# Forrest-Z/my-lidar-graph-slam

Hardware: AMD Instinct MI355X
Metric: scans/sec + p50 scan-match ms, 1081-beam vs 1000×1000@5cm grid, 1/2/4/8 GPU (higher is better)
Workload: dtype f64

## Files before the change

### include/lgs_hip.h

```cpp
#ifndef LGS_HIP_H
#define LGS_HIP_H

#include <stddef.h>
#include <stdint.h>

#ifdef __cplusplus
extern "C" {
#endif

#define LGS_ABI_VERSION 2

#define LGS_OK               0
#define LGS_ERR_INVALID_ARG  1
#define LGS_ERR_HIP          2
#define LGS_ERR_NO_DEVICE    3
#define LGS_ERR_OOM          4
#define LGS_ERR_INTERNAL     5

typedef struct lgs_ctx  lgs_ctx;
typedef struct lgs_grid lgs_grid;
typedef struct lgs_scan lgs_scan;

typedef struct { double x, y, theta; } lgs_pose2d;

// ... 64 lines not shown
#define LGS_OPT_SORT_BARRIER_US 23
#define LGS_OPT_FINE_STAGED   24
#define LGS_OPT_SMALL_WINDOW  25
#define LGS_OPT_POST_RECORDS  26
#define LGS_OPT_FUSED_PLANES  27
#define LGS_OPT_PRIORITY_TAIL 28
#define LGS_OPT_HV_FULL       29
#define LGS_OPT_SPLIT_CHUNKS  30
#define LGS_OPT_DEVICE_HITS   31
#define LGS_OPT_SEED_WIDE     32
#define LGS_OPT_ZERO_TILES    33
#define LGS_OPT_DEVICE_TIMING 34
#define LGS_OPT_LEAN_PROJECT  35
#define LGS_OPT_PGCG_GRID_NODES 36
#define LGS_OPT_FAST_ROWS     37
#define LGS_OPT_HV_INZERO     38
#define LGS_OPT_POISON_WS     15
int  lgs_ctx_set_option(lgs_ctx* ctx, int option, double value);

int  lgs_debug_item_buffer(lgs_ctx* ctx, int item, int which, void* out, size_t cap, size_t* bytes);

int  lgs_debug_libm(lgs_ctx* ctx, int op, const double* x, int n, double* out);

int  lgs_debug_keysort(lgs_ctx* ctx, const unsigned* keys, unsigned* out, long long n, int lo, int bits);

int  lgs_debug_copy_counters(const lgs_ctx* ctx, long long* direct, long long* staged);

int  lgs_debug_offset_checks(lgs_ctx* ctx, int reset, unsigned long long* out);

typedef struct {
// ... 468 lines not shown
```

### my-lidar-graph-slam_amd/csrc/k_rtcsm.hip

```cpp
#include "lgs_internal.hpp"
#include "loop_host.hpp"
#include "fast_cell.hpp"
#include "hv_zero.hpp"
#include "sq_cost_stage.hpp"
#include "ge_cost_device.hpp"

#include <algorithm>
#include <cfloat>
#include <cstring>
#include <map>
#include <mutex>
#include <thread>
#include <type_traits>

using namespace lgs;

namespace lgs {
void launch_precompute(lgs_ctx* ctx, const lgs_grid* in, int win, double* out, const PlaneGeom* planes);
void launch_precompute_jobs(lgs_ctx* ctx, const PrecompJob* d_jobs, int njobs, int maxW, int maxH, int win);
bool precompute_planes_ok(const lgs_grid* in, int win);
void precompute_tile_grid(int maxW, int maxH, int win, int njobs, int* gx, int* gy, int* rows);
}

namespace {
// ... 14 lines not shown
    const double* cmap;
    const SuperT* super;
    const int* negflag;
    int pgen;
    int gen;
    RtcsmRecord* rec;
    int* keepc;
    int2* idx;
    int* cbase;
    int* tedge;
    double* cscore;
    uint8_t* cflag;
    int* list;
    int* segcnt;
    int nseg;
    int* dlist;
    int* nsel;
    int frows;
    double* fval;
    int* fpos;
    double* part_c;
    long long* part_k;
    int nparts;
    double* Lp;
    double* Lc;
    double* seedm;
    int nseedm;
    double* sbound;
    double* poses7;
    int4* cidx;
// ... 1561 lines not shown
                    if (q.x - pl.win_x < 0 || q.y - pl.win_y < 0)
                        unsafe |= strip_read(cmap, q.x + x0, q.y + y0, pl, ext);
                }
            }
        }
        if (active) {
            it.cflag[k] = (unsafe && (sum + ext) * pl.sb_mult >= L) ? 1 : 0;
        }
    }
}

struct WorkList {
    int* cnt;
    int* sbl;
    int* al;
    int region, tmax;
};
constexpr int kListMaxNv = 4096;
#ifndef LGS_LIST_WAVES
#define LGS_LIST_WAVES 4096
#endif
constexpr int kListWaves = LGS_LIST_WAVES;
#ifndef LGS_LIST_XCD
#define LGS_LIST_XCD 1
#endif
#ifndef LGS_XCD2
#define LGS_XCD2 1
#endif
static_assert(kListWaves % 8 == 0, "whole workgroups per XCD");
constexpr int kUnsafeGroups = 4096;

__global__ __launch_bounds__(64) void k_keep(Items items, WorkList W, DevTs dts)
// ... 4 lines not shown
    const RtcsmPlan& pl = it.pl;
    const int t = blockIdx.x;
    if (t >= pl.T) return;
    const int lane = threadIdx.x;
    const int nsb2 = pl.nsbx * pl.nsby;
    double L = -INFINITY;
#pragma unroll
    for (int b = 0; b < kSeedCands; ++b) L = fmax(L, it.Lc[b]);
    if (t == 0 && lane == 0) *it.Lp = L;
    bool kp = false;
    if (lane < nsb2) {
        const double bnd = it.sbound[(size_t)t * nsb2 + lane];
        kp = (bnd > pl.thr) && bnd >= L;
    }
    const unsigned long long bal = __ballot(kp);
    if (!bal) return;
    int base = 0;
    if (lane == 0) {
        unsigned long long nb = 0;
        for (unsigned long long mm = bal; mm; mm &= mm - 1) {
            const int sb = __ffsll((long long)mm) - 1;
            const int a = sb % pl.nsbx, b = sb / pl.nsbx;
            nb += (unsigned long long)(min(kSB, pl.ncx - kSB * a) * min(kSB, pl.ncy - kSB * b));
        }
        atomicAdd(&it.rec->coarse_evals, nb);
        base = atomicAdd(W.cnt + 16 * j, __popcll(bal));
        if (it.tedge[t] == it.gen) W.al[(size_t)j * W.tmax + atomicAdd(W.cnt + 16 * j + 1, 1)] = t;
    }
    base = __shfl(base, 0, 64);
    if (kp) W.sbl[(size_t)j * W.region + base + __popcll(bal & ((1ull << lane) - 1ull))] = t << 6 | lane;
}

__device__ __forceinline__ int list_prefix(const WorkList& W, int which, int n, int& c)
{
    const int lane = threadIdx.x & 63;
    c = lane < n ? W.cnt[16 * lane + which] : 0;
#pragma unroll
    for (int off = 1; off < 64; off <<= 1) {
        const int u = __shfl_up(c, off, 64);
        if (lane >= off) c += u;
    }
    return __shfl(c, 63, 64);
// ... 109 lines not shown
        }
        if (active) {
            const long long k = (long long)t * pl.P + (long long)jx * pl.ncy + jy;
            it.cscore[k] = sum;
            it.cflag[k] = 0;
        }
    }
}

__global__ __launch_bounds__(64 * kLaneWaves) void k_unsafe_list(Items items, WorkList W, int n,
                                                                 const double* __restrict__ zero, DevTs dts)
{
    const DtsScope dts_scope(dts);
    const int lane = threadIdx.x & 63;
    int c;
    const int total = list_prefix(W, 1, n, c);
    for (int a = blockIdx.x; a < total; a += gridDim.x) {
        const int j = __popcll(__ballot(lane < n && c <= a));
        const int cprev = __shfl(c, max(j - 1, 0), 64);
        const int before = j > 0 ? cprev : 0;
        unsafe_angle(items[j], W.al[(size_t)j * W.tmax + (a - before)]);
    }
}

__device__ void eval_block(const RtcsmPlan& pl, const double* __restrict__ grid,
                           const int2* __restrict__ idx, const double* __restrict__ zero,
                           long long k, int2* sidx, double& f, int& pos)
{
    const int tt = (int)(k / pl.P);
    const int rem = (int)(k % pl.P);
    const int jx = rem / pl.ncy, jy = rem % pl.ncy;
// ... 324 lines not shown
            if (k[r] == bk) v[r] = -INFINITY, k[r] = LLONG_MAX;
    }
    return pick;
}
__global__ __launch_bounds__(kSeedMembersThreads) void k_seed_members(Items items, DevTs dts)
{
#if LGS_XCD2
    const Blk sbk = xcd_block();
#else
    const Blk sbk{ (int)blockIdx.x, (int)blockIdx.y, (int)blockIdx.z };
#endif
    const DtsScope dts_scope(dts);
    const MatchItem& it = items[sbk.y];
    const RtcsmPlan& pl = it.pl;
    const double* __restrict__ cmap = it.cmap;
    if (sbk.x == 0 && threadIdx.x < 2 && it.keepc) it.keepc[threadIdx.x] = 0;
    extern __shared__ char smem[];
    __shared__ double red[2][kSeedMembersThreads / 64][16];
    __shared__ long long s_cand;
    const int tid = threadIdx.x, lane = tid & 63, w = tid >> 6;
    const int nsb2 = pl.nsbx * pl.nsby;
    const int Nv = pl.Nv;
    if (w == 0) {
        const long long pick = seed_pick_wave(it, pl, (int)sbk.x);
        if (lane == 0) s_cand = pick;
    }
    __syncthreads();
    double* out = it.seedm + 3 * sbk.x;
    const long long ck = s_cand;
    if (ck == LLONG_MAX) {
        if (tid == 0) {
// ... 79 lines not shown
#if LGS_XCD2
    const Blk sbk = xcd_block();
#else
    const Blk sbk{ (int)blockIdx.x, (int)blockIdx.y, (int)blockIdx.z };
#endif
    const DtsScope dts_scope(dts);
    const MatchItem& it = items[sbk.y];
    const RtcsmPlan& pl = it.pl;
    const double* __restrict__ grid = it.grid;
    const double* __restrict__ cmap = it.cmap;
    const double* __restrict__ part_c = it.part_c;
    const long long* __restrict__ part_k = it.part_k;
    const int nparts = it.nparts;
    double* __restrict__ Lc = it.Lc;
    RtcsmRecord* rec = it.rec;
    if (MODE == 0 && sbk.x == 0 && threadIdx.x < 2 && it.keepc) it.keepc[threadIdx.x] = 0;
    extern __shared__ char smem[];
    __shared__ double sv[16];
    __shared__ long long sk[16];
    __shared__ long long cand[kSeedCands];
    __shared__ double red[1024];
    __shared__ double reda[1024];
    const int tid = threadIdx.x;
    const int nsb2 = pl.nsbx * pl.nsby;
    const int Nv = pl.Nv;
    LGS_PROBE_DECL;
    LGS_PROBE_MARK();
    double Lmine = -INFINITY;
    if constexpr (MODE == 2) {
        if (tid < 64) {
            const bool ok = tid < it.nseedm;
// ... 152 lines not shown
            }
        }
        __syncthreads();
        Lmine = seed_fine(pl, grid, zero, sidx, sk[0], sv[1], sv[2], red, reda, sv);
        LGS_PROBE_MARK();
    }
    if (tid == 0) {
        Lc[sbk.x] = Lmine;
        if (sbk.x == 0) rec->coarse_evals = 0ull;
    }
    LGS_PROBE_MARK();
    LGS_PROBE_PRINT("seed(b0: cand, members, argmax, stage, fine, reduce, publish)");
}

constexpr int kSelSeg = 1024;

template <int kSelThreads>
__global__ __launch_bounds__(kSelThreads) void k_select(Items items, int use_sbound, DevTs dts)
{
    const DtsScope dts_scope(dts);
    static_assert(kSelSeg % kSelThreads == 0 && kSelThreads % 64 == 0, "whole chunks of whole waves");
    const MatchItem& it = items[blockIdx.y];
    if ((int)blockIdx.x >= it.nseg) return;
    const RtcsmPlan& pl = it.pl;
    const double* __restrict__ cscore = it.cscore;
    const uint8_t* __restrict__ cflag = it.cflag;
    const double* __restrict__ sbound = use_sbound ? it.sbound : nullptr;
    int* __restrict__ list = it.list;
    int* __restrict__ segcnt = it.segcnt;
    constexpr int kW = kSelThreads / 64, kChunks = kSelSeg / kSelThreads;
    __shared__ int s_w[kChunks][kW];
    const double L = *it.Lp;
    const int lane = threadIdx.x & 63, wid = threadIdx.x >> 6;
    bool f[kChunks];
#pragma unroll
    for (int j = 0; j < kChunks; ++j) {
// ... 22 lines not shown
        const unsigned long long bal = __ballot(f[j]);
        int o = off;
        for (int w = 0; w < wid; ++w) o += s_w[j][w];
        if (f[j]) list[(size_t)blockIdx.x * kSelSeg + o + __popcll(bal & ((1ull << lane) - 1ull))] =
            (int)((long long)blockIdx.x * kSelSeg + j * kSelThreads + threadIdx.x);
        for (int w = 0; w < kW; ++w) off += s_w[j][w];
    }
    if (threadIdx.x == 0) segcnt[blockIdx.x] = off;
}

__device__ void seg_prefix(const int* __restrict__ segcnt, int nseg, int* pref, int* ws)
{
    const int nt = blockDim.x, tid = threadIdx.x, lane = tid & 63, wid = tid >> 6;
    const int chunk = (nseg + nt - 1) / nt;
    const int lo = min(tid * chunk, nseg), hi = min(lo + chunk, nseg);
    int c = 0;
    for (int i = lo; i < hi; ++i) c += segcnt[i];
    int incl = c;
    for (int off = 1; off < 64; off <<= 1) {
        const int t = __shfl_up(incl, off, 64);
        if (lane >= off) incl += t;
    }
    const int last = min(63, nt - 1 - wid * 64);
    if (lane == last) ws[wid] = incl;
    __syncthreads();
    int run = incl - c;
    for (int j = 0; j < wid; ++j) run += ws[j];
    for (int i = lo; i < hi; ++i) {
        pref[i] = run;
        run += segcnt[i];
    }
    if (tid == nt - 1) pref[nseg] = run;
    __syncthreads();
}

__device__ __forceinline__ int seg_of(const int* pref, int nseg, int b)
{
    int lo = 0, hi = nseg;
    while (hi - lo > 1) {
        const int mid = (lo + hi) >> 1;
        if (pref[mid] <= b) lo = mid;
        else hi = mid;
    }
    return lo;
}
// ... 14 lines not shown
    int* __restrict__ fpos = it_.fpos;
    extern __shared__ char smem[];
    __shared__ double sv[16];
    __shared__ long long sk[16];
    __shared__ int ws[16];
    int* pref = (int*)(smem + eval_smem);
    LGS_PROBE_DECL;
    LGS_PROBE_MARK();
    seg_prefix(segcnt, nseg, pref, ws);
    LGS_PROBE_MARK();
    const int n = pref[nseg];
    constexpr int R = LR > 0 ? LR : 1;
    for (int it = wg.x; it < n * R; it += gridDim.x) {
        const int b = it / R;
        const int sg = seg_of(pref, nseg, b);
        const long long k = list[(size_t)sg * kSelSeg + (b - pref[sg])];
        double f;
        int pos;
        if constexpr (LR > 0)
            eval_block_t<LR, kFineDepth>(pl, grid, idx, zero, k, smem, sv, sk, f, pos, it % R);
        else
            eval_block(pl, grid, idx, zero, k, (int2*)smem, f, pos);
        if (threadIdx.x == 0) {
            fval[it] = f;
            fpos[it] = pos;
        }
        LGS_PROBE_MARK();
    }
    LGS_PROBE_PRINT("fine(seg_prefix, item0[, item1])");
}

__global__ __launch_bounds__(256) void k_compact(Items items)
{
    const MatchItem& it = items[blockIdx.x];
    extern __shared__ int pref[];
    __shared__ int ws[16];
    seg_prefix(it.segcnt, it.nseg, pref, ws);
    const int lane = threadIdx.x & 63, w = threadIdx.x >> 6;
    for (int sg = w; sg < it.nseg; sg += 4) {
        const int c = pref[sg + 1] - pref[sg];
        const int* __restrict__ src = it.list + (size_t)sg * kSelSeg;
        int* __restrict__ dst = it.dlist + pref[sg];
        for (int i = lane; i < c; i += 64) dst[i] = src[i];
    }
    if (threadIdx.x == 0) *it.nsel = pref[it.nseg];
}

constexpr int kFineLanesWaves = 1;
constexpr int kFineLanesMaxNv = 2048;
__global__ __launch_bounds__(64 * kFineLanesWaves) void k_fine_lanes(Items items, int n,
                                                                    const double* __restrict__ zero)
{
    __shared__ int ipref[kMaxBatchItems + 1];
    extern __shared__ int2 sidx[];
    if (threadIdx.x < 64) {
        const int j = threadIdx.x;
        const int c = (j < n) ? *items[j].nsel : 0;
        int incl = c;
        for (int off = 1; off < 64; off <<= 1) {
            const int t = __shfl_up(incl, off, 64);
// ... 208 lines not shown
    seg_prefix(segcnt, nseg, pref, ws);
    const int n = pref[nseg];
    const double L = *Lp;
    const int lane = threadIdx.x;
    double s = pl.thr;
    long long bestk = -1;
    int bestpos = 0;
    bool dangerous = false;
    for (int b0 = 0; b0 < n; b0 += 64) {
        const int b = b0 + lane;
        double c = -INFINITY, f = -INFINITY;
        long long k = -1;
        int pos = 0;
        if (b < n) {
            const int sg = seg_of(pref, nseg, b);
            k = list[(size_t)sg * kSelSeg + (b - pref[sg])];
            c = cscore[k];
            const size_t fi = (size_t)b * frows;
            f = fval[fi];
            pos = fpos[fi];
            for (int r = 1; r < frows; ++r) {
                const double fr = fval[fi + r];
                const int pr = fpos[fi + r];
                if (fr > f || (fr == f && pr < pos)) {
                    f = fr;
                    pos = pr;
                }
            }
            if (cflag[k] && c < L && f >= L) dangerous = true;
        }
        const int cnt = min(64, n - b0);
// ... 753 lines not shown
    int P = 0, nsb2 = 0, chunks = 0, low_res = 0, cb = 0;
    bool pair = false;
    bool oct = false;
    int unit8 = 2;
    int nsby = 0;
    bool pruned = false;
    bool small = false;
    bool lr5 = false;
    bool fine_lanes = false;
    bool fine_staged = false;
    int frows = 1;
    int kernel_size = 0;
    bool sq = false;
    bool gx = false;
    WorkList wl{};
};

inline int item_nparts(const BatchShape& B, const RtcsmPlan& pl, bool pruned)
{
    return pruned ? B.chunks * pl.T : ((B.P + B.cb - 1) / B.cb) * pl.T;
}

inline bool uses_super(const lgs_ctx* ctx, int nv_max, int nsb2, bool dense)
{
    return !(dense || ctx->force_dense) && ctx->super_prune && nv_max <= kSeedMaxNv &&
           nsb2 <= 64 && nsb2 >= ctx->prune_min_super;
}

struct ItemLayout {
    size_t idx, cbase, cscore, cflag, list, segcnt, dlist, fval, fpos, part_c, part_k, sbound, poses7, cidx,
        terms, count, btab, atab, total;
};
ItemLayout item_layout(int Tmax, int NvMax, int P, int nsb2, int chunks, int cb, int frows, int Nmax)
{
    ItemLayout L{};
    size_t o = 0;
    auto take = [&](size_t bytes) {
        const size_t r = o;
        o += align256(std::max<size_t>(bytes, 16));
        return r;
    };
    const size_t K = (size_t)Tmax * P;
    const size_t nidx = (size_t)Tmax * std::max(NvMax, 1) + kPad;
    const size_t nseg = (K + kSelSeg - 1) / kSelSeg;
    const size_t nparts = std::max<size_t>((size_t)((P + cb - 1) / cb) * Tmax, (size_t)chunks * Tmax);
    L.idx = take(sizeof(int2) * nidx);
    L.cbase = take(sizeof(int) * 2 * nidx);
    L.cscore = take(sizeof(double) * K);
    L.cflag = take(K);
    L.list = take(sizeof(int) * nseg * kSelSeg);
    L.segcnt = take(sizeof(int) * nseg);
    L.dlist = take(sizeof(int) * K);
    L.fval = take(sizeof(double) * K * frows);
    L.fpos = take(sizeof(int) * K * frows);
    L.part_c = take(sizeof(double) * nparts);
    L.part_k = take(sizeof(long long) * nparts);
    L.sbound = take(sizeof(double) * (size_t)Tmax * std::max(nsb2, 1));
    L.poses7 = take(sizeof(double) * 21);
    L.cidx = take(sizeof(int4) * 7 * (size_t)Nmax);
    L.terms = take(sizeof(double) * 7 * (size_t)Nmax);
    L.count = take(128 + 24 * kSeedWide);
    L.btab = take(sizeof(double4) * (size_t)std::max(NvMax, 1));
    L.atab = take(sizeof(double2) * (size_t)std::max(Tmax, 1));
    L.total = o;
    return L;
}

void bind_workspace(MatchItem& it, char* base, const ItemLayout& L, int frows)
{
    it.idx = (int2*)(base + L.idx);
    it.cbase = (int*)(base + L.cbase);
    it.cscore = (double*)(base + L.cscore);
    it.cflag = (uint8_t*)(base + L.cflag);
    it.list = (int*)(base + L.list);
    it.segcnt = (int*)(base + L.segcnt);
    it.fval = (double*)(base + L.fval);
    it.fpos = (int*)(base + L.fpos);
    it.part_c = (double*)(base + L.part_c);
    it.part_k = (long long*)(base + L.part_k);
    it.sbound = (double*)(base + L.sbound);
    it.poses7 = (double*)(base + L.poses7);
    it.cidx = (int4*)(base + L.cidx);
    it.terms = (double*)(base + L.terms);
    it.Lp = (double*)(base + L.count);
    it.Lc = (double*)(base + L.count + 64);
    it.nsel = (int*)(base + L.count + 64 + 8 * kSeedCands);
    it.seedm = (double*)(base + L.count + 128);
    it.dlist = (int*)(base + L.dlist);
    it.btab = (double4*)(base + L.btab);
    it.atab = (double2*)(base + L.atab);
    static_assert(64 + 8 * kSeedCands + 4 <= 128, "count block layout");
    it.frows = frows;
    it.nseg = (int)((it.pl.K + kSelSeg - 1) / kSelSeg);
}

inline size_t plane_bytes(const RtcsmPlan& pl)
{
    return align256(sizeof(double) * (size_t)pl.low_res * pl.low_res * (size_t)pl.pstride);
}
inline size_t plane16_bytes(const RtcsmPlan& pl)
{
    return align256(sizeof(unsigned short) * (size_t)pl.low_res * pl.low_res * (size_t)pl.pstride) + 256;
}
inline size_t set_bytes(const RtcsmPlan& pl) { return plane_bytes(pl) + plane16_bytes(pl); }
inline size_t super_bytes(const RtcsmPlan& pl)
{
    if (pl.oct) return align256(4 * (size_t)pl.unit8 * pl.low_res * pl.low_res * (size_t)pl.pstrideO);
    return align256(sizeof(SuperT) * (size_t)pl.low_res * pl.low_res * (size_t)pl.pstride4);
// ... 557 lines not shown
            ctx->timing_end(tok);
            LGS_HIP_CHECK(hipGetLastError());
        }
        const int tok = ctx->timing_begin(K_SEED, 8.0 * B.low_res * B.low_res * (double)B.NvMax * n);
        if (B.lr5)
            hipLaunchKernelGGL(k_seed<5>, dim3(1, n), dim3(64 * 5), eval_t_smem<5>(B.NvMax), st, d_items, zero,
                               dense ? 1 : 0);
        else
            hipLaunchKernelGGL(k_seed<0>, dim3(1, n), dim3(64), sidx_bytes(B.NvMax), st, d_items, zero,
                               dense ? 1 : 0);
        ctx->timing_end(tok);
        LGS_HIP_CHECK(hipGetLastError());
    }
    {
        const int tok_ = ctx->timing_begin(K_SELECT, 10.0 * (double)B.Tmax * B.P * n);
        if (!ctx->skipped(K_SELECT)) {
            if (n >= ctx->lanes_min_batch)
                hipLaunchKernelGGL(HIP_KERNEL_NAME(k_select<256>), dim3((unsigned)B.nsegMax, n), dim3(256), 0, st,
                                   d_items, B.pruned ? 1 : 0, ctx->dts(tok_));
            else
                hipLaunchKernelGGL(HIP_KERNEL_NAME(k_select<kSelSeg>), dim3((unsigned)B.nsegMax, n), dim3(kSelSeg), 0,
                                   st, d_items, B.pruned ? 1 : 0, ctx->dts(tok_));
        }
        ctx->timing_end(tok_);
        LGS_HIP_CHECK(hipGetLastError());
    }
    if (B.fine_lanes) {
        hipLaunchKernelGGL(k_compact, dim3(n), dim3(256), pref_bytes(B.nsegMax), st, d_items);
        LGS_HIP_CHECK(hipGetLastError());
        const int tok_ = ctx->timing_begin(K_FINE, 0.0);
        if (ctx->skipped(K_FINE)) {
        } else if (B.fine_staged && ctx->fine_staged) {
            hipLaunchKernelGGL(k_fine_regs, dim3(4096), dim3(64), sizeof(unsigned) * (size_t)(B.NvMax + kFrPad), st,
                               d_items, n, zero, ctx->dts(tok_));
        } else {
            hipLaunchKernelGGL(k_fine_lanes, dim3(4096), dim3(64 * kFineLanesWaves),
                               sizeof(int2) * (size_t)(B.NvMax + 4 * kPipe), st, d_items, n, zero);
// ... 292 lines not shown
    B.oct = p0.oct != 0;
    B.unit8 = p0.unit8;
    B.nsby = p0.nsby;
    B.pruned = uses_super(ctx, B.NvMax, B.nsb2, false);
    B.lr5 = lr5_path(B.NvMax, B.low_res);
    B.fine_lanes = n >= ctx->lanes_min_batch && B.low_res * B.low_res <= 64 &&
                   B.NvMax <= kFineLanesMaxNv;
    B.frows = (B.lr5 && !B.fine_lanes) ? 5 : 1;
    B.fine_staged = B.fine_lanes && B.low_res == 5;
    for (int j = 0; j < n && B.fine_staged; ++j)
        B.fine_staged = grids[j]->w % 2 == 0 && ((uintptr_t)grids[j]->d & 15) == 0 && grids[j]->w <= 8192 &&
                        grids[j]->h <= 8192;
    B.kernel_size = cost->kernel_size;
    B.sq = sq != nullptr;
    B.gx = alt.gx;
    B.nsegMax = (int)(((long long)B.Tmax * B.P + kSelSeg - 1) / kSelSeg);
    B.small = ctx->small_window && !ctx->force_dense && p0.P == 1 && B.low_res >= 2 && B.low_res <= 7 &&
              B.NvMax <= kSmallMaxNv && n <= kTedgeCtrs;
    for (int j = 0; j < n; ++j) B.small = B.small && grids[j]->w >= B.low_res && grids[j]->h >= 1;
    for (auto& s : sets) B.small = B.small && !s.coarse;
    if (B.small) B.pruned = false;
    if (B.pruned && n >= ctx->lanes_min_batch && B.NvMax <= kListMaxNv && B.Tmax < (1 << 24) && B.nsb2 <= 64) {
        int region = 1;
        for (auto& it : items) region = std::max(region, it.pl.T * it.pl.nsbx * it.pl.nsby);
        int* wl = (int*)ctx->ensure(S_KEEP, sizeof(int) * (size_t)n * (16 + (size_t)region + (size_t)B.Tmax));
        B.wl = WorkList{ wl, wl + 16 * (size_t)n, wl + 16 * (size_t)n + (size_t)region * n, region, B.Tmax };
    }
    const ItemLayout L = item_layout(B.Tmax, B.NvMax, B.P, B.nsb2, B.chunks, B.cb, B.frows, Nmax);
    char* ws = (char*)ctx->ensure(ctx->banked(S_BATCH_WS), L.total * (size_t)n);
    RtcsmRecord* d_rec = (RtcsmRecord*)ctx->ensure(ctx->banked(S_RECORDS), sizeof(RtcsmRecord) * (size_t)n);
    const size_t rec_bytes = sizeof(RtcsmRecord) * (size_t)n;
    constexpr size_t kDtsBytes = sizeof(unsigned long long) * 2 * kDtsSub * kDtsSlots;
    RtcsmRecord* h_rec = (RtcsmRecord*)ctx->ensure_pinned_rec(align256(rec_bytes) + 256 + kDtsBytes);
    unsigned* h_flag = (unsigned*)((char*)h_rec + align256(rec_bytes));
    F.id = ++ctx->timing_batch;
    struct DtsScope {
        lgs_ctx* c;
        ~DtsScope() { c->dts_dev = nullptr; }
    } dts_scope{ ctx };
    if (ctx->profile && ctx->dev_timing) {
        unsigned long long*& db = ctx->dts_buf[ctx->bank];
        if (++ctx->dts_gen >= (1u << 24) || !db) {
// ... 8 lines not shown
        ctx->dts_used = 0;
    }
    if (ctx->poison_ws) {
        LGS_HIP_CHECK(hipMemsetAsync(ws, 0xFF, L.total * (size_t)n, ctx->stream));
        LGS_HIP_CHECK(hipMemsetAsync(d_rec, 0xFF, sizeof(RtcsmRecord) * (size_t)n, ctx->stream));
    }
    int* tedge = ctx->tedge_buffer((size_t)n * B.Tmax);
    int* sctr = B.small ? ctx->small_counters((size_t)n * B.Tmax) : nullptr;
    Upload up(ctx);
    scans_to_device(ctx, scans, n, &up);
    const SetJobs sj = B.small ? SetJobs{} : build_sets(ctx, p0, sets, B.pruned, up);
    std::vector<int> gens((size_t)n);
    for (int j = 0; j < n; ++j) {
        MatchItem& it = items[j];
        bind_workspace(it, ws + L.total * (size_t)j, L, B.frows);
        it.tedge = tedge + (size_t)j * B.Tmax;
        it.grid = grids[j]->d;
        it.ranges = scans[j]->d_ranges;
        it.angles = scans[j]->d_angles;
        const PlaneSet& s = sets[set_of[j]];
        it.cmap = s.cmap;
        it.super = s.super;
        it.negflag = s.negflag;
        it.pgen = s.pgen;
        it.gen = gens[j] = ctx->generation = ctx->next_stamp();
        it.rec = d_rec + j;
        it.keepc = B.wl.cnt ? B.wl.cnt + 16 * j : sctr ? sctr + j : nullptr;
        it.nparts = item_nparts(B, it.pl, B.pruned);
        it.nseedm = std::min(ctx->seed_wide, kSeedWide);
        it.inject = ctx->inject_index ? 1 : 0;
// ... 15 lines not shown
                               sizeof(int2) * (size_t)q.T * q.Nv, sizeof(double) * (size_t)q.K };
        lgs_ctx::DbgItem& d = ctx->dbg[j];
        for (int k = 0; k < 8; ++k) {
            d.buf[k] = b[k];
            d.bytes[k] = sz[k];
        }
        d.buf[8] = ij.cmap;
        d.bytes[8] = ij.cmap ? plane_bytes(q) : 0;
        d.buf[9] = ij.super;
        d.bytes[9] = ij.super ? super_bytes(q) : 0;
        const PlaneSet* dps = B.small ? nullptr : &sets[set_of[j]];
        d.buf[10] = dps ? dps->hv_in : nullptr;
        d.bytes[10] = dps ? dps->hv_in_bytes : 0;
        d.buf[11] = dps ? dps->hv_out : nullptr;
        d.bytes[11] = dps ? dps->hv_out_bytes : 0;
        d.gen = ij.gen;
    }
    const size_t items_off = up.append(items.data(), items.size());
    up.flush();
    if (!B.small) launch_sets(ctx, p0, sets, sj, up);
    struct StreamRestore {
        lgs_ctx* c;
        hipStream_t s;
        ~StreamRestore() { c->stream = s; }
    } restore{ ctx, ctx->stream };
    if (!B.small && ctx->prio_tail && ctx->hi) {
        LGS_HIP_CHECK(hipEventRecord(ctx->split_ev[ctx->bank], ctx->stream));
        LGS_HIP_CHECK(hipStreamWaitEvent(ctx->hi, ctx->split_ev[ctx->bank], 0));
        ctx->stream = ctx->hi;
    }
// ... 110 lines not shown
                                host_cost_cells(cp, scans[j], P7[pi], b, cells);
                                cpatch.push_back(make_int4(pi * cp.N + b, 0, 0, 0));
                                cpatch.push_back(make_int4(cells[0], cells[1], cells[2], cells[3]));
                            }
                    }
                    opt.cost_patches = &cpatch;
                    opt.cost_only = true;
                    rerun = true;
                    fixups = 1;
                }
            }
            if (!rerun) break;
            BatchShape B1 = B;
            B1.n = 1;
            B1.Tmax = items[j].pl.T;
            B1.nsegMax = items[j].nseg;
            B1.pruned = pruned = !B.small && uses_super(ctx, B.NvMax, B.nsb2, opt.dense);
            std::vector<MatchItem> one(1, items[j]);
            one[0].nparts = item_nparts(B1, one[0].pl, B1.pruned);
            one[0].lean = 0;
            const int g = one[0].gen = ctx->generation = ctx->next_stamp();
            if ((size_t)j < ctx->dbg.size()) ctx->dbg[j].gen = g;
            Upload u1(ctx);
            const size_t off = u1.append(one.data(), 1);
            u1.flush();
            enqueue_items(ctx, B1, u1.at<MatchItem>(off), one, opt);
            LGS_HIP_CHECK(hipMemcpyAsync(&h_rec[j], d_rec + j, sizeof(RtcsmRecord), hipMemcpyDeviceToHost,
                                         ctx->stream));
            ctx->sync();
            if (ctx->profile) ctx->harvest_upto(F.id);
            rec = HostRecord(h_rec[j], g);
            if (opt.patches || opt.host_idx) rec.guard_count = 0;
        }
// ... 168 lines not shown
        out[j].normalized_cost = c[0] / (double)scans[j]->n;
        out[j].estimated_pose = move_backward(best[j], scans[j]->rel);
        const double dl = grid->res, da = 1e-2;
        const double g[3] = { 0.5 * (c[1] - c[2]) / dl, 0.5 * (c[3] - c[4]) / dl, 0.5 * (c[5] - c[6]) / da };
        for (int a = 0; a < 3; ++a)
            for (int b = 0; b < 3; ++b) out[j].covariance[3 * a + b] = g[a] * g[b];
        out[j].covariance[0] += 0.01;
        out[j].covariance[4] += 0.01;
        out[j].covariance[8] += 0.01;
    }
}
}

extern "C" int lgs_debug_item_buffer(lgs_ctx* ctx, int item, int which, void* out, size_t cap, size_t* bytes)
{
    if (!ctx || which < 0 || which >= 12 || item < 0) return LGS_ERR_INVALID_ARG;
    return guarded(ctx, [&] {
        LGS_REQUIRE((size_t)item < ctx->dbg.size(), "no such item in the last correlative batch");
        const lgs_ctx::DbgItem& d = ctx->dbg[(size_t)item];
        const size_t n = d.bytes[which];
        if (bytes) *bytes = n;
        if (!out || cap == 0) return;
        const size_t k = std::min(cap, n);
        LGS_HIP_CHECK(hipSetDevice(ctx->device));
        ctx->sync();
        LGS_HIP_CHECK(hipMemcpy(out, d.buf[which], k, hipMemcpyDeviceToHost));
        if (which == 4) {
            int* f = (int*)out;
            for (size_t i = 0; i < k / sizeof(int); ++i) f[i] = f[i] == d.gen ? 1 : 0;
        }
    });
// ... 608 lines not shown
```

### my-lidar-graph-slam_amd/csrc/lgs_core.hip

```cpp
#include "lgs_internal.hpp"
#include "hv_zero.hpp"

#include <atomic>
#include <condition_variable>
#include <cstring>
#include <mutex>
#include <thread>

#include <pthread.h>

using namespace lgs;

void* lgs_ctx::ensure(int slot, size_t bytes)
{
    if (bytes == 0) bytes = 16;
    if (buf_bytes[slot] >= bytes) return buf[slot];
    if (buf[slot]) {
        LGS_HIP_CHECK(hipStreamSynchronize(stream));
        LGS_HIP_CHECK(hipFree(buf[slot]));
        buf[slot] = nullptr;
        buf_bytes[slot] = 0;
    }
    size_t want = bytes + bytes / 4;
    void* p = nullptr;
// ... 491 lines not shown
    case LGS_OPT_PRUNE_MIN_SUPER: ctx->prune_min_super = (int)value; return LGS_OK;
    case LGS_OPT_COOP_TILES: ctx->coop_tiles = (long long)value; return LGS_OK;
    case LGS_OPT_FINE_STAGED: ctx->fine_staged = value != 0.0; return LGS_OK;
    case LGS_OPT_SMALL_WINDOW: ctx->small_window = value != 0.0; return LGS_OK;
    case LGS_OPT_POST_RECORDS: ctx->post_records = value != 0.0; return LGS_OK;
    case LGS_OPT_FUSED_PLANES: ctx->fused_planes = value != 0.0; return LGS_OK;
    case LGS_OPT_PRIORITY_TAIL: ctx->prio_tail = value != 0.0; return LGS_OK;
    case LGS_OPT_DEVICE_TIMING: ctx->dev_timing = value != 0.0; return LGS_OK;
    case LGS_OPT_HV_FULL: ctx->hv_full = value != 0.0; return LGS_OK;
    case LGS_OPT_SPLIT_CHUNKS: ctx->split_chunks = value != 0.0; return LGS_OK;
    case LGS_OPT_DEVICE_HITS: ctx->device_hits = value != 0.0; return LGS_OK;
    case LGS_OPT_ZERO_TILES: ctx->zero_tiles = value != 0.0; return LGS_OK;
    case LGS_OPT_HV_INZERO: ctx->hv_inzero = value != 0.0; return LGS_OK;
    case LGS_OPT_LEAN_PROJECT: ctx->lean_project = value != 0.0; return LGS_OK;
    case LGS_OPT_FAST_ROWS: ctx->fast_rows = value != 0.0; return LGS_OK;
    case LGS_OPT_PGCG_GRID_NODES:
        if (!(value >= 0.0)) return LGS_ERR_INVALID_ARG;
        ctx->pg_grid_nodes = (int)std::min(value, 2147483647.0);
        return LGS_OK;
    case LGS_OPT_LOOP_SEARCH_MIN_PAIRS:
        if (!(value >= 0.0)) return LGS_ERR_INVALID_ARG;
        ctx->loop_min_pairs = (long long)std::min(value, 9.0e18);
        return LGS_OK;
    case LGS_OPT_LOOP_SEARCH_GROUP:
        if (!(value >= 0.0)) return LGS_ERR_INVALID_ARG;
        ctx->loop_group = (int)std::min(value, 134217728.0);
        return LGS_OK;
    case LGS_OPT_SEED_WIDE:
        if (!(value >= 0.0 && value <= 16.0)) return LGS_ERR_INVALID_ARG;
        ctx->seed_wide = (int)value;
// ... 1039 lines not shown
```

### my-lidar-graph-slam_amd/csrc/lgs_internal.hpp

```cpp
#pragma once

#include <hip/hip_runtime.h>

#include <climits>
#include <cmath>
#include <cstdint>
#include <cstring>
#include <functional>
#include <stdexcept>
#include <string>
#include <type_traits>
#include <memory>
#include <map>
#include <mutex>
#include <atomic>
#include <condition_variable>
#include <utility>
#include <vector>

#include "lgs_hip.h"
#include "lgs_error.hpp"
#include "pose_host.hpp"

namespace lgs {
// ... 235 lines not shown
    long long handoff_spin_us = 200000;
#ifndef LGS_FINE_STAGED_DEFAULT
#define LGS_FINE_STAGED_DEFAULT 1
#endif
    bool fine_staged = LGS_FINE_STAGED_DEFAULT;
    long long coop_tiles = -1;
    long long sort_barrier_us = 50000;
    long long handoff_fallbacks = 0;
    bool peer_staged = false;
    int prune_min_super = 1;
    bool small_window = true;
    bool fused_planes = true;
    int seed_wide = 12;
    bool lean_project = true;
    bool fast_rows = true;
    bool zero_tiles = true;
    bool device_hits = true;
    bool split_chunks = false;
    bool hv_inzero = true;
    bool hv_full = false;
    bool prio_tail = false;
    hipStream_t hi = nullptr;
    hipEvent_t split_ev[2] = {};
    bool post_records = true;
    long long copies_direct = 0, copies_staged = 0;
    int lanes_min_batch = 2;
    long long ray_chunk_keys = 1LL << 28;
    int next_stamp();
    unsigned skip_mask = 0;
    bool skipped(int kernel) const { return (skip_mask >> kernel) & 1u; }
    bool poison_ws = false;
    struct DbgItem {
        const void* buf[12];
        size_t bytes[12];
        int gen;
    };
    std::vector<DbgItem> dbg;
    int generation = 0;
    void* buf[lgs::S_NUM_SLOTS] = {};
    size_t buf_bytes[lgs::S_NUM_SLOTS] = {};
    void* pinned = nullptr;
    size_t pinned_bytes = 0;
    void* pinned_up = nullptr;
    size_t pinned_up_bytes = 0;
    void* pinned_up_b = nullptr;
    size_t pinned_up_b_bytes = 0;
    bool up_busy[2] = { false, false };
    void* pinned_rec[2] = {};
    size_t pinned_rec_bytes[2] = {};
// ... 431 lines not shown
```

### my-lidar-graph-slam_amd/lgs_amd/abi.py

```python
from __future__ import annotations

import ctypes as C
import os
from collections import namedtuple
from typing import Optional, Sequence

import numpy as np

_HERE = os.path.dirname(os.path.abspath(__file__))
LIB_PATH = os.path.join(_HERE, "liblgs_hip.so")

LGS_OK = 0
LGS_OPT_GUARD_EPS = 1
LGS_OPT_FORCE_DENSE = 2
LGS_OPT_INJECT_INDEX = 3
LGS_OPT_GUARD_CAP = 4
LGS_OPT_PROFILE = 5
LGS_OPT_PROFILE_MASK = 7
LGS_OPT_SPIN_SYNC = 8
LGS_OPT_SUPER_PRUNE = 9
LGS_OPT_LANES_MIN_BATCH = 11
LGS_OPT_RAY_CHUNK_KEYS = 13
LGS_OPT_POISON_WS = 15
LGS_OPT_SKIP_MASK = 10
# ... 13 lines not shown
LGS_OPT_DEVICE_HITS = 31
LGS_OPT_SEED_WIDE = 32
LGS_OPT_ZERO_TILES = 33
LGS_OPT_DEVICE_TIMING = 34
LGS_OPT_LEAN_PROJECT = 35
LGS_OPT_PGCG_GRID_NODES = 36
LGS_OPT_FAST_ROWS = 37
LGS_OPT_HV_INZERO = 38
KERNEL_IDS = ["k_project", "k_coarse", "k_seed", "k_select", "k_fine", "k_replay", "k_cost", "k_precompute",
              "k_linsolve", "k_ray_emit", "k_ray_apply", "k_super", "k_super_planes", "k_bb_score",
              "k_bb_expand", "k_coarse_aux", "k_match_small", "k_gs_score",
              "k_cost_sq", "k_cost_gx"]
MORE_KERNEL_IDS = ["k_loop_search"]
LGS_OPT_LOOP_SEARCH_MIN_PAIRS = 39
LGS_OPT_LOOP_SEARCH_GROUP = 40


class Pose2D(C.Structure):
    _fields_ = [("x", C.c_double), ("y", C.c_double), ("theta", C.c_double)]

    def tuple(self):
        return (self.x, self.y, self.theta)


class ScanHost(C.Structure):
    _fields_ = [
        ("ranges", C.POINTER(C.c_double)),
        ("angles", C.POINTER(C.c_double)),
        ("n", C.c_int),
        ("rel_sensor_pose", Pose2D),
# ... 1066 lines not shown
        self.check(self.lib.lgs_maps_construct_from_scans(self.h, mh, lo, hi, nm, arr, ps, n, C.byref(bp)),
                   "maps_construct_from_scans")

    def construct_global_map(self, res: float, patch_size: int, scans, poses, bp: "BuilderParams") -> "Map":
        n = len(scans)
        arr = (_P * n)(*[s.h for s in scans])
        ps = (Pose2D * n)(*[Pose2D(*p) for p in poses])
        h = _P()
        self.check(self.lib.lgs_map_construct_global(self.h, res, patch_size, arr, ps, n, C.byref(bp), C.byref(h)),
                   "map_construct_global")
        return Map(self, h)

    DEBUG_BUFFERS = {"sbound": (0, np.float64), "part_c": (1, np.float64), "part_k": (2, np.int64),
                     "L": (3, np.float64), "tedge": (4, np.int32), "cbase": (5, np.int32), "idx": (6, np.int32),
                     "cscore": (7, np.float64), "planes": (8, np.float64), "super": (9, np.float16),
                     "hv_inmask": (10, np.uint64), "hv_outmask": (11, np.uint64)}

    def debug_buffer(self, name: str, item: int = 0) -> np.ndarray:
        which, dt = self.DEBUG_BUFFERS[name]
        n = C.c_size_t()
        self.check(self.lib.lgs_debug_item_buffer(self.h, item, which, None, 0, C.byref(n)), "debug_item_buffer")
        out = np.zeros(n.value // np.dtype(dt).itemsize, dtype=dt)
        self.check(self.lib.lgs_debug_item_buffer(self.h, item, which, out.ctypes.data_as(_P), out.nbytes,
                                                  C.byref(n)),
                   "debug_item_buffer")
        return out

    def debug_libm(self, op: int, x) -> np.ndarray:
        x = np.ascontiguousarray(x, dtype=np.float64)
        out = np.zeros((len(x), 2) if op == 0 else len(x), dtype=np.float64)
        self.check(self.lib.lgs_debug_libm(self.h, op, x.ctypes.data_as(_P), len(x), out.ctypes.data_as(_P)),
# ... 268 lines not shown
```

Measured before the change: 106,000.

## Select fine candidates per kept angle using super-block keep masks

```diff
diff --git a/include/lgs_hip.h b/include/lgs_hip.h
--- a/include/lgs_hip.h
+++ b/include/lgs_hip.h
@@ -102,6 +102,7 @@
 #define LGS_OPT_LEAN_PROJECT  35
 #define LGS_OPT_PGCG_GRID_NODES 36
 #define LGS_OPT_FAST_ROWS     37
+#define LGS_OPT_SELECT_ANGLES 41
 #define LGS_OPT_HV_INZERO     38
 #define LGS_OPT_POISON_WS     15
 int  lgs_ctx_set_option(lgs_ctx* ctx, int option, double value);
diff --git a/my-lidar-graph-slam_amd/csrc/k_rtcsm.hip b/my-lidar-graph-slam_amd/csrc/k_rtcsm.hip
--- a/my-lidar-graph-slam_amd/csrc/k_rtcsm.hip
+++ b/my-lidar-graph-slam_amd/csrc/k_rtcsm.hip
@@ -52,6 +52,8 @@
     int* list;
     int* segcnt;
     int nseg;
+    int segstride;
+    unsigned long long* keepm;
     int* dlist;
     int* nsel;
     int frows;
@@ -1643,8 +1645,10 @@
     int* cnt;
     int* sbl;
     int* al;
+    int* kl;
     int region, tmax;
 };
+constexpr int kListCtrs = 3;
 constexpr int kListMaxNv = 4096;
 #ifndef LGS_LIST_WAVES
 #define LGS_LIST_WAVES 4096
@@ -1679,6 +1683,10 @@
         kp = (bnd > pl.thr) && bnd >= L;
     }
     const unsigned long long bal = __ballot(kp);
+    if (W.kl && lane == 0) {
+        it.keepm[t] = bal;
+        if (!bal) it.segcnt[t] = 0;
+    }
     if (!bal) return;
     int base = 0;
     if (lane == 0) {
@@ -1689,8 +1697,11 @@
             nb += (unsigned long long)(min(kSB, pl.ncx - kSB * a) * min(kSB, pl.ncy - kSB * b));
         }
         atomicAdd(&it.rec->coarse_evals, nb);
-        base = atomicAdd(W.cnt + 16 * j, __popcll(bal));
-        if (it.tedge[t] == it.gen) W.al[(size_t)j * W.tmax + atomicAdd(W.cnt + 16 * j + 1, 1)] = t;
+        const unsigned long long both =
+            atomicAdd((unsigned long long*)(W.cnt + 16 * j), (1ull << 32) | (unsigned long long)__popcll(bal));
+        base = (int)(unsigned)both;
+        if (W.kl) W.kl[(size_t)j * W.tmax + (int)(both >> 32)] = t;
+        if (it.tedge[t] == it.gen) W.al[(size_t)j * W.tmax + atomicAdd(W.cnt + 16 * j + 2, 1)] = t;
     }
     base = __shfl(base, 0, 64);
     if (kp) W.sbl[(size_t)j * W.region + base + __popcll(bal & ((1ull << lane) - 1ull))] = t << 6 | lane;
@@ -1830,7 +1841,7 @@
     const DtsScope dts_scope(dts);
     const int lane = threadIdx.x & 63;
     int c;
-    const int total = list_prefix(W, 1, n, c);
+    const int total = list_prefix(W, 2, n, c);
     for (int a = blockIdx.x; a < total; a += gridDim.x) {
         const int j = __popcll(__ballot(lane < n && c <= a));
         const int cprev = __shfl(c, max(j - 1, 0), 64);
@@ -2185,7 +2196,7 @@
     const MatchItem& it = items[sbk.y];
     const RtcsmPlan& pl = it.pl;
     const double* __restrict__ cmap = it.cmap;
-    if (sbk.x == 0 && threadIdx.x < 2 && it.keepc) it.keepc[threadIdx.x] = 0;
+    if (sbk.x == 0 && threadIdx.x < kListCtrs && it.keepc) it.keepc[threadIdx.x] = 0;
     extern __shared__ char smem[];
     __shared__ double red[2][kSeedMembersThreads / 64][16];
     __shared__ long long s_cand;
@@ -2295,7 +2306,7 @@
     const int nparts = it.nparts;
     double* __restrict__ Lc = it.Lc;
     RtcsmRecord* rec = it.rec;
-    if (MODE == 0 && sbk.x == 0 && threadIdx.x < 2 && it.keepc) it.keepc[threadIdx.x] = 0;
+    if (MODE == 0 && sbk.x == 0 && threadIdx.x < kListCtrs && it.keepc) it.keepc[threadIdx.x] = 0;
     extern __shared__ char smem[];
     __shared__ double sv[16];
     __shared__ long long sk[16];
@@ -2478,12 +2489,68 @@
 }
 
 constexpr int kSelSeg = 1024;
+constexpr int kSelMaxAngles = 7 * 1024;
+constexpr int kSelGroups = 2048;
 
 template <int kSelThreads>
-__global__ __launch_bounds__(kSelThreads) void k_select(Items items, int use_sbound, DevTs dts)
+__device__ __forceinline__ void select_angles(Items items, const WorkList& W, int n)
+{
+    constexpr int kW = kSelThreads / 64;
+    __shared__ int s_a[2][kW];
+    const int lane = threadIdx.x & 63, wid = threadIdx.x >> 6;
+    int c;
+    const int total = list_prefix(W, 1, n, c);
+    int par = 0;
+    for (int a = blockIdx.x; a < total; a += gridDim.x) {
+        const int j = __builtin_amdgcn_readfirstlane(__popcll(__ballot(lane < n && c <= a)));
+        const int cprev = __shfl(c, max(j - 1, 0), 64);
+        const int before = __builtin_amdgcn_readfirstlane(j > 0 ? cprev : 0);
+        const MatchItem& it = items[j];
+        const RtcsmPlan& pl = it.pl;
+        const int t = __builtin_amdgcn_readfirstlane(W.kl[(size_t)j * W.tmax + (a - before)]);
+        const unsigned long long km = it.keepm[t];
+        const double L = *it.Lp;
+        const int P = pl.P, ncy = pl.ncy, nsbx = pl.nsbx;
+        const int base = t * P;
+        const double* __restrict__ cscore = it.cscore + base;
+        const uint8_t* __restrict__ cflag = it.cflag + base;
+        int* __restrict__ list = it.list + base;
+        int off = 0;
+        for (int i0 = 0; i0 < P; i0 += kSelThreads, par ^= 1) {
+            const int i = i0 + (int)threadIdx.x;
+            bool f = false;
+            if (i < P) {
+                const int jx = i / ncy, jy = i - jx * ncy;
+                if ((km >> ((jy / kSB) * nsbx + jx / kSB)) & 1ull) {
+                    const double cs = cscore[i];
+                    f = (cs > pl.thr) && (cflag[i] || cs >= L);
+                }
+            }
+            const unsigned long long bal = __ballot(f);
+            if (lane == 0) s_a[par][wid] = __popcll(bal);
+            __syncthreads();
+            int o = off;
+#pragma unroll
+            for (int w = 0; w < kW; ++w) {
+                const int cw = s_a[par][w];
+                if (w < wid) o += cw;
+                off += cw;
+            }
+            if (f) list[o + __popcll(bal & ((1ull << lane) - 1ull))] = base + i;
+        }
+        if (threadIdx.x == 0) it.segcnt[t] = off;
+    }
+}
+
+template <int kSelThreads>
+__global__ __launch_bounds__(kSelThreads) void k_select(Items items, int use_sbound, WorkList W, int n, DevTs dts)
 {
     const DtsScope dts_scope(dts);
     static_assert(kSelSeg % kSelThreads == 0 && kSelThreads % 64 == 0, "whole chunks of whole waves");
+    if (W.kl) {
+        select_angles<kSelThreads>(items, W, n);
+        return;
+    }
     const MatchItem& it = items[blockIdx.y];
     if ((int)blockIdx.x >= it.nseg) return;
     const RtcsmPlan& pl = it.pl;
@@ -2536,8 +2603,18 @@
     const int nt = blockDim.x, tid = threadIdx.x, lane = tid & 63, wid = tid >> 6;
     const int chunk = (nseg + nt - 1) / nt;
     const int lo = min(tid * chunk, nseg), hi = min(lo + chunk, nseg);
+    constexpr int kRegs = 8;
+    const bool regs = chunk <= kRegs;
+    int v[kRegs];
     int c = 0;
-    for (int i = lo; i < hi; ++i) c += segcnt[i];
+    if (regs) {
+#pragma unroll
+        for (int k = 0; k < kRegs; ++k) v[k] = lo + k < hi ? segcnt[lo + k] : 0;
+#pragma unroll
+        for (int k = 0; k < kRegs; ++k) c += v[k];
+    } else {
+        for (int i = lo; i < hi; ++i) c += segcnt[i];
+    }
     int incl = c;
     for (int off = 1; off < 64; off <<= 1) {
         const int t = __shfl_up(incl, off, 64);
@@ -2548,9 +2625,17 @@
     __syncthreads();
     int run = incl - c;
     for (int j = 0; j < wid; ++j) run += ws[j];
-    for (int i = lo; i < hi; ++i) {
-        pref[i] = run;
-        run += segcnt[i];
+    if (regs) {
+#pragma unroll
+        for (int k = 0; k < kRegs; ++k) {
+            if (lo + k < hi) pref[lo + k] = run;
+            run += v[k];
+        }
+    } else {
+        for (int i = lo; i < hi; ++i) {
+            pref[i] = run;
+            run += segcnt[i];
+        }
     }
     if (tid == nt - 1) pref[nseg] = run;
     __syncthreads();
@@ -2595,7 +2680,7 @@
     for (int it = wg.x; it < n * R; it += gridDim.x) {
         const int b = it / R;
         const int sg = seg_of(pref, nseg, b);
-        const long long k = list[(size_t)sg * kSelSeg + (b - pref[sg])];
+        const long long k = list[(size_t)sg * it_.segstride + (b - pref[sg])];
         double f;
         int pos;
         if constexpr (LR > 0)
@@ -2617,14 +2702,12 @@
     extern __shared__ int pref[];
     __shared__ int ws[16];
     seg_prefix(it.segcnt, it.nseg, pref, ws);
-    const int lane = threadIdx.x & 63, w = threadIdx.x >> 6;
-    for (int sg = w; sg < it.nseg; sg += 4) {
-        const int c = pref[sg + 1] - pref[sg];
-        const int* __restrict__ src = it.list + (size_t)sg * kSelSeg;
-        int* __restrict__ dst = it.dlist + pref[sg];
-        for (int i = lane; i < c; i += 64) dst[i] = src[i];
-    }
-    if (threadIdx.x == 0) *it.nsel = pref[it.nseg];
+    const int n = pref[it.nseg];
+    for (int b = threadIdx.x; b < n; b += 256) {
+        const int sg = seg_of(pref, it.nseg, b);
+        it.dlist[b] = it.list[(size_t)sg * it.segstride + (b - pref[sg])];
+    }
+    if (threadIdx.x == 0) *it.nsel = n;
 }
 
 constexpr int kFineLanesWaves = 1;
@@ -2863,7 +2946,7 @@
         int pos = 0;
         if (b < n) {
             const int sg = seg_of(pref, nseg, b);
-            k = list[(size_t)sg * kSelSeg + (b - pref[sg])];
+            k = list[(size_t)sg * it.segstride + (b - pref[sg])];
             c = cscore[k];
             const size_t fi = (size_t)b * frows;
             f = fval[fi];
@@ -3647,6 +3730,7 @@
     bool sq = false;
     bool gx = false;
     WorkList wl{};
+    bool sel_angles = false;
 };
 
 inline int item_nparts(const BatchShape& B, const RtcsmPlan& pl, bool pruned)
@@ -3660,8 +3744,23 @@
            nsb2 <= 64 && nsb2 >= ctx->prune_min_super;
 }
 
+inline bool select_by_angle(const lgs_ctx* ctx, const BatchShape& B)
+{
+    return ctx->select_angles && B.pruned && B.n >= ctx->lanes_min_batch && B.wl.cnt && !ctx->skipped(K_COARSE) &&
+           B.Tmax <= kSelMaxAngles;
+}
+inline void set_segments(MatchItem& it, bool by_angle)
+{
+    it.segstride = by_angle ? it.pl.P : kSelSeg;
+    it.nseg = by_angle ? it.pl.T : (int)((it.pl.K + kSelSeg - 1) / kSelSeg);
+}
+inline int max_segments(const BatchShape& B)
+{
+    return B.sel_angles ? B.Tmax : (int)(((long long)B.Tmax * B.P + kSelSeg - 1) / kSelSeg);
+}
+
 struct ItemLayout {
-    size_t idx, cbase, cscore, cflag, list, segcnt, dlist, fval, fpos, part_c, part_k, sbound, poses7, cidx,
+    size_t idx, cbase, cscore, cflag, list, segcnt, keepm, dlist, fval, fpos, part_c, part_k, sbound, poses7, cidx,
         terms, count, btab, atab, total;
 };
 ItemLayout item_layout(int Tmax, int NvMax, int P, int nsb2, int chunks, int cb, int frows, int Nmax)
@@ -3682,7 +3781,8 @@
     L.cscore = take(sizeof(double) * K);
     L.cflag = take(K);
     L.list = take(sizeof(int) * nseg * kSelSeg);
-    L.segcnt = take(sizeof(int) * nseg);
+    L.segcnt = take(sizeof(int) * std::max(nseg, (size_t)Tmax));
+    L.keepm = take(sizeof(unsigned long long) * (size_t)Tmax);
     L.dlist = take(sizeof(int) * K);
     L.fval = take(sizeof(double) * K * frows);
     L.fpos = take(sizeof(int) * K * frows);
@@ -3707,6 +3807,7 @@
     it.cflag = (uint8_t*)(base + L.cflag);
     it.list = (int*)(base + L.list);
     it.segcnt = (int*)(base + L.segcnt);
+    it.keepm = (unsigned long long*)(base + L.keepm);
     it.fval = (double*)(base + L.fval);
     it.fpos = (int*)(base + L.fpos);
     it.part_c = (double*)(base + L.part_c);
@@ -3724,7 +3825,7 @@
     it.atab = (double2*)(base + L.atab);
     static_assert(64 + 8 * kSeedCands + 4 <= 128, "count block layout");
     it.frows = frows;
-    it.nseg = (int)((it.pl.K + kSelSeg - 1) / kSelSeg);
+    set_segments(it, false);
 }
 
 inline size_t plane_bytes(const RtcsmPlan& pl)
@@ -4312,13 +4413,17 @@
     }
     {
         const int tok_ = ctx->timing_begin(K_SELECT, 10.0 * (double)B.Tmax * B.P * n);
+        WorkList none{};
         if (!ctx->skipped(K_SELECT)) {
-            if (n >= ctx->lanes_min_batch)
+            if (B.sel_angles)
+                hipLaunchKernelGGL(HIP_KERNEL_NAME(k_select<256>), dim3(std::min(kSelGroups, n * B.Tmax)), dim3(256), 0,
+                                   st, d_items, 1, B.wl, n, ctx->dts(tok_));
+            else if (n >= ctx->lanes_min_batch)
                 hipLaunchKernelGGL(HIP_KERNEL_NAME(k_select<256>), dim3((unsigned)B.nsegMax, n), dim3(256), 0, st,
-                                   d_items, B.pruned ? 1 : 0, ctx->dts(tok_));
+                                   d_items, B.pruned ? 1 : 0, none, n, ctx->dts(tok_));
             else
                 hipLaunchKernelGGL(HIP_KERNEL_NAME(k_select<kSelSeg>), dim3((unsigned)B.nsegMax, n), dim3(kSelSeg), 0,
-                                   st, d_items, B.pruned ? 1 : 0, ctx->dts(tok_));
+                                   st, d_items, B.pruned ? 1 : 0, none, n, ctx->dts(tok_));
         }
         ctx->timing_end(tok_);
         LGS_HIP_CHECK(hipGetLastError());
@@ -4641,7 +4746,6 @@
     B.kernel_size = cost->kernel_size;
     B.sq = sq != nullptr;
     B.gx = alt.gx;
-    B.nsegMax = (int)(((long long)B.Tmax * B.P + kSelSeg - 1) / kSelSeg);
     B.small = ctx->small_window && !ctx->force_dense && p0.P == 1 && B.low_res >= 2 && B.low_res <= 7 &&
               B.NvMax <= kSmallMaxNv && n <= kTedgeCtrs;
     for (int j = 0; j < n; ++j) B.small = B.small && grids[j]->w >= B.low_res && grids[j]->h >= 1;
@@ -4650,9 +4754,13 @@
     if (B.pruned && n >= ctx->lanes_min_batch && B.NvMax <= kListMaxNv && B.Tmax < (1 << 24) && B.nsb2 <= 64) {
         int region = 1;
         for (auto& it : items) region = std::max(region, it.pl.T * it.pl.nsbx * it.pl.nsby);
-        int* wl = (int*)ctx->ensure(S_KEEP, sizeof(int) * (size_t)n * (16 + (size_t)region + (size_t)B.Tmax));
-        B.wl = WorkList{ wl, wl + 16 * (size_t)n, wl + 16 * (size_t)n + (size_t)region * n, region, B.Tmax };
-    }
+        int* wl = (int*)ctx->ensure(S_KEEP, sizeof(int) * (size_t)n * (16 + (size_t)region + 2 * (size_t)B.Tmax));
+        int* al = wl + 16 * (size_t)n + (size_t)region * n;
+        B.wl = WorkList{ wl, wl + 16 * (size_t)n, al, nullptr, region, B.Tmax };
+        B.sel_angles = select_by_angle(ctx, B);
+        if (B.sel_angles) B.wl.kl = al + (size_t)B.Tmax * n;
+    }
+    B.nsegMax = max_segments(B);
     const ItemLayout L = item_layout(B.Tmax, B.NvMax, B.P, B.nsb2, B.chunks, B.cb, B.frows, Nmax);
     char* ws = (char*)ctx->ensure(ctx->banked(S_BATCH_WS), L.total * (size_t)n);
     RtcsmRecord* d_rec = (RtcsmRecord*)ctx->ensure(ctx->banked(S_RECORDS), sizeof(RtcsmRecord) * (size_t)n);
@@ -4691,6 +4799,7 @@
     for (int j = 0; j < n; ++j) {
         MatchItem& it = items[j];
         bind_workspace(it, ws + L.total * (size_t)j, L, B.frows);
+        set_segments(it, B.sel_angles);
         it.tedge = tedge + (size_t)j * B.Tmax;
         it.grid = grids[j]->d;
         it.ranges = scans[j]->d_ranges;
@@ -4736,6 +4845,10 @@
         d.bytes[10] = dps ? dps->hv_in_bytes : 0;
         d.buf[11] = dps ? dps->hv_out : nullptr;
         d.bytes[11] = dps ? dps->hv_out_bytes : 0;
+        d.buf[12] = ij.segcnt;
+        d.bytes[12] = sizeof(int) * (size_t)ij.nseg;
+        d.buf[13] = ij.keepm;
+        d.bytes[13] = B.sel_angles ? sizeof(unsigned long long) * (size_t)q.T : 0;
         d.gen = ij.gen;
     }
     const size_t items_off = up.append(items.data(), items.size());
@@ -4876,9 +4989,12 @@
             BatchShape B1 = B;
             B1.n = 1;
             B1.Tmax = items[j].pl.T;
-            B1.nsegMax = items[j].nseg;
             B1.pruned = pruned = !B.small && uses_super(ctx, B.NvMax, B.nsb2, opt.dense);
+            B1.sel_angles = select_by_angle(ctx, B1);
+            if (!B1.sel_angles) B1.wl.kl = nullptr;
+            B1.nsegMax = max_segments(B1);
             std::vector<MatchItem> one(1, items[j]);
+            set_segments(one[0], B1.sel_angles);
             one[0].nparts = item_nparts(B1, one[0].pl, B1.pruned);
             one[0].lean = 0;
             const int g = one[0].gen = ctx->generation = ctx->next_stamp();
@@ -5077,7 +5193,7 @@
 
 extern "C" int lgs_debug_item_buffer(lgs_ctx* ctx, int item, int which, void* out, size_t cap, size_t* bytes)
 {
-    if (!ctx || which < 0 || which >= 12 || item < 0) return LGS_ERR_INVALID_ARG;
+    if (!ctx || which < 0 || which >= 14 || item < 0) return LGS_ERR_INVALID_ARG;
     return guarded(ctx, [&] {
         LGS_REQUIRE((size_t)item < ctx->dbg.size(), "no such item in the last correlative batch");
         const lgs_ctx::DbgItem& d = ctx->dbg[(size_t)item];
diff --git a/my-lidar-graph-slam_amd/csrc/lgs_core.hip b/my-lidar-graph-slam_amd/csrc/lgs_core.hip
--- a/my-lidar-graph-slam_amd/csrc/lgs_core.hip
+++ b/my-lidar-graph-slam_amd/csrc/lgs_core.hip
@@ -529,6 +529,7 @@
     case LGS_OPT_HV_INZERO: ctx->hv_inzero = value != 0.0; return LGS_OK;
     case LGS_OPT_LEAN_PROJECT: ctx->lean_project = value != 0.0; return LGS_OK;
     case LGS_OPT_FAST_ROWS: ctx->fast_rows = value != 0.0; return LGS_OK;
+    case LGS_OPT_SELECT_ANGLES: ctx->select_angles = value != 0.0; return LGS_OK;
     case LGS_OPT_PGCG_GRID_NODES:
         if (!(value >= 0.0)) return LGS_ERR_INVALID_ARG;
         ctx->pg_grid_nodes = (int)std::min(value, 2147483647.0);
diff --git a/my-lidar-graph-slam_amd/csrc/lgs_internal.hpp b/my-lidar-graph-slam_amd/csrc/lgs_internal.hpp
--- a/my-lidar-graph-slam_amd/csrc/lgs_internal.hpp
+++ b/my-lidar-graph-slam_amd/csrc/lgs_internal.hpp
@@ -273,6 +273,7 @@
     int seed_wide = 12;
     bool lean_project = true;
     bool fast_rows = true;
+    bool select_angles = true;
     bool zero_tiles = true;
     bool device_hits = true;
     bool split_chunks = false;
@@ -290,8 +291,8 @@
     bool skipped(int kernel) const { return (skip_mask >> kernel) & 1u; }
     bool poison_ws = false;
     struct DbgItem {
-        const void* buf[12];
-        size_t bytes[12];
+        const void* buf[14];
+        size_t bytes[14];
         int gen;
     };
     std::vector<DbgItem> dbg;
diff --git a/my-lidar-graph-slam_amd/lgs_amd/abi.py b/my-lidar-graph-slam_amd/lgs_amd/abi.py
--- a/my-lidar-graph-slam_amd/lgs_amd/abi.py
+++ b/my-lidar-graph-slam_amd/lgs_amd/abi.py
@@ -51,6 +51,7 @@
 MORE_KERNEL_IDS = ["k_loop_search"]
 LGS_OPT_LOOP_SEARCH_MIN_PAIRS = 39
 LGS_OPT_LOOP_SEARCH_GROUP = 40
+LGS_OPT_SELECT_ANGLES = 41
 
 
 class Pose2D(C.Structure):
@@ -1147,7 +1148,8 @@
     DEBUG_BUFFERS = {"sbound": (0, np.float64), "part_c": (1, np.float64), "part_k": (2, np.int64),
                      "L": (3, np.float64), "tedge": (4, np.int32), "cbase": (5, np.int32), "idx": (6, np.int32),
                      "cscore": (7, np.float64), "planes": (8, np.float64), "super": (9, np.float16),
-                     "hv_inmask": (10, np.uint64), "hv_outmask": (11, np.uint64)}
+                     "hv_inmask": (10, np.uint64), "hv_outmask": (11, np.uint64),
+                     "segcnt": (12, np.int32), "keepm": (13, np.uint64)}
 
     def debug_buffer(self, name: str, item: int = 0) -> np.ndarray:
         which, dt = self.DEBUG_BUFFERS[name]
```

Result: faster. 108,000, median of 5 (+1.9%).
